# SamuelSchlesinger/anonymous-credit-tokens

Hardware: AMD Instinct MI355X
Metric: spend-proof verifies/sec (whole node), batch=2^20 (higher is better)
Workload: dtype u32 limbs / u64 accumulators (integer)

## Files before the change

anonymous-credit-tokens_amd/csrc/msm.h:

```cpp
#pragma once
#include "ge25519.h"

namespace act {

#ifndef ACT_FB_WBITS
#define ACT_FB_WBITS 16
#endif
constexpr int FB_WBITS = ACT_FB_WBITS;
constexpr int FB_WINDOWS = (253 + FB_WBITS - 1) / FB_WBITS;
constexpr int FB_ENTRIES = 1 << FB_WBITS;
constexpr int NIELS_WORDS = 32;
constexpr size_t FB_TABLE_WORDS = (size_t)FB_WINDOWS * FB_ENTRIES * NIELS_WORDS;

ACT_HD ge_niels niels_load(const uint32_t* p) {
  ge_niels n;
#if defined(__HIP_DEVICE_COMPILE__)
  const uint4* q = reinterpret_cast<const uint4*>(p);
  uint4 a[7];
  for (int i = 0; i < 7; i++) a[i] = q[i];
  uint32_t w[28];
  for (int i = 0; i < 7; i++) { w[4 * i] = a[i].x; w[4 * i + 1] = a[i].y; w[4 * i + 2] = a[i].z; w[4 * i + 3] = a[i].w; }
  for (int i = 0; i < FE_LIMBS; i++) { n.ypx.v[i] = w[i]; n.ymx.v[i] = w[FE_LIMBS + i]; n.xy2d.v[i] = w[2 * FE_LIMBS + i]; }
#else
  for (int i = 0; i < FE_LIMBS; i++) { n.ypx.v[i] = p[i]; n.ymx.v[i] = p[FE_LIMBS + i]; n.xy2d.v[i] = p[2 * FE_LIMBS + i]; }
#endif
  return n;
}
ACT_HD void niels_store(uint32_t* p, const ge_niels& n) {
  for (int i = 0; i < FE_LIMBS; i++) { p[i] = n.ypx.v[i]; p[FE_LIMBS + i] = n.ymx.v[i]; p[2 * FE_LIMBS + i] = n.xy2d.v[i]; }
  for (int i = 3 * FE_LIMBS; i < NIELS_WORDS; i++) p[i] = 0;
}
ACT_HD ge_niels niels_from_affine(const ge& p) {
  ge_niels n;
  n.ypx = fe_carry(fe_add(p.Y, p.X));
  n.ymx = fe_carry(fe_sub(p.Y, p.X));
  n.xy2d = fe_mul(p.T, fe_d2());
  return n;
}
constexpr int GE_WORDS = 4 * FE_LIMBS;
ACT_HD void ge_words(uint32_t w[GE_WORDS], const ge& g) {
  for (int i = 0; i < FE_LIMBS; i++) { w[i] = g.X.v[i]; w[FE_LIMBS + i] = g.Y.v[i]; w[2 * FE_LIMBS + i] = g.Z.v[i]; w[3 * FE_LIMBS + i] = g.T.v[i]; }
}
ACT_HD ge ge_of_words(const uint32_t w[GE_WORDS]) {
  ge g;
  for (int i = 0; i < FE_LIMBS; i++) { g.X.v[i] = w[i]; g.Y.v[i] = w[FE_LIMBS + i]; g.Z.v[i] = w[2 * FE_LIMBS + i]; g.T.v[i] = w[3 * FE_LIMBS + i]; }
  return g;
}
ACT_HD void ge_store(uint32_t* p, const ge& g) { ge_words(p, g); }
ACT_HD ge ge_load(const uint32_t* p) { return ge_of_words(p); }

struct FbTab { const uint32_t* p; uint32_t wbits; uint32_t id; };
ACT_HD uint32_t fb_windows(uint32_t wbits) { return (253u + wbits - 1u) / wbits; }
ACT_HD size_t fb_table_words(uint32_t wbits) { return (size_t)fb_windows(wbits) * ((size_t)1 << wbits) * NIELS_WORDS; }

ACT_HD ge_niels fb_table_entry(ge b, uint32_t wbits, uint32_t gid) {
  uint32_t pos = gid >> wbits, e = gid & ((1u << wbits) - 1u);
  for (uint32_t i = 0; i < wbits * pos; i++) b = ge_double(b);
  ge acc = ge_identity();
  ge_cached bc = ge_to_cached(b);
  for (int bit = (int)wbits - 1; bit >= 0; bit--) {
    acc = ge_double(acc);
    if ((e >> bit) & 1u) acc = ge_add_cached(acc, bc);
  }
  fe zi = fe_invert(acc.Z);
  ge af; af.X = fe_mul(acc.X, zi); af.Y = fe_mul(acc.Y, zi); af.Z = fe_one(); af.T = fe_mul(af.X, af.Y);
  return niels_from_affine(af);
}

ACT_HD uint32_t fb_next_digit(uint32_t w[8], uint32_t wbits) {
  uint32_t digit = w[0] & ((1u << wbits) - 1u);
  for (int i = 0; i < 7; i++) w[i] = (w[i] >> wbits) | (w[i + 1] << (32u - wbits));
  w[7] >>= wbits;
  return digit;
}
ACT_HD ge fixed_base_acc(ge acc, const FbTab& t, const sc& s) {
  fe_count_fixed_base(t.id);
  uint32_t w[8];
  for (int i = 0; i < 8; i++) w[i] = s.v[i];
  const uint32_t nw = fb_windows(t.wbits);
  const size_t entries = (size_t)1 << t.wbits;
  ge_niels cur = niels_load(t.p + (size_t)fb_next_digit(w, t.wbits) * NIELS_WORDS);
  for (uint32_t pos = 1; pos < nw; pos++) {
    ge_niels nxt = niels_load(t.p + ((size_t)pos * entries + fb_next_digit(w, t.wbits)) * NIELS_WORDS);
    acc = ge_madd(acc, cur);
    cur = nxt;
  }
  return ge_madd(acc, cur);
}

struct digit4 { bool nonzero, two, neg; };
ACT_HD digit4 next_digit4(uint32_t w[8], uint32_t& carry) {
  uint32_t v = (w[0] & 3u) + carry;
  for (int i = 0; i < 7; i++) w[i] = (w[i] >> 2) | (w[i + 1] << 30);
  w[7] >>= 2;
  digit4 d;
  carry = v >= 3u ? 1u : 0u;
  d.nonzero = (v != 0u) && (v != 4u);
  d.two = (v == 2u);
  d.neg = (v == 3u);
  return d;
}
ACT_HD ge chain_step_add(const ge& acc, const ge_cached& c1, const ge_cached& c2, const digit4& d) {
  ge_cached q;
  uint32_t m2 = fe_mask(d.two);
  q.YpX = fe_select_m(c1.YpX, c2.YpX, m2);
  q.YmX = fe_select_m(c1.YmX, c2.YmX, m2);
  q.Z = fe_select_m(c1.Z, c2.Z, m2);
  q.T2d = fe_select_m(c1.T2d, c2.T2d, m2);
  q = ge_cached_cneg(q, d.neg);
  return ge_add_cached(acc, q);
}
template <int NACC>
ACT_HD void chain(ge* acc, const ge& N, const sc* s) {
  uint32_t w[NACC][8], carry[NACC];
  for (int a = 0; a < NACC; a++) { carry[a] = 0; for (int i = 0; i < 8; i++) w[a][i] = s[a].v[i]; }
  ge P = N;
  for (int step = 0; step < 127; step++) {
    ge_cached c1 = ge_to_cached(P);
    ge Q = ge_double(P);
    ge_cached c2 = ge_to_cached(Q);
    if (step < 126) P = ge_double(Q);
#pragma unroll
    for (int a = 0; a < NACC; a++) {
      digit4 d = next_digit4(w[a], carry[a]);
      if (d.nonzero) acc[a] = chain_step_add(acc[a], c1, c2, d);
    }
  }
}

struct naf_state { uint32_t w[9]; };
ACT_HD naf_state naf_init(const sc& s) { naf_state n; for (int i = 0; i < 8; i++) n.w[i] = s.v[i]; n.w[8] = 0; return n; }
ACT_HD int naf_next(naf_state& n) {
  int d = 0;
  if (n.w[0] & 1u) {
    d = 2 - (int)(n.w[0] & 3u);
    if (d < 0) {
      uint64_t c = 1;
      for (int i = 0; i < 9; i++) { c += n.w[i]; n.w[i] = (uint32_t)c; c >>= 32; }
    } else {
      n.w[0] &= ~1u;
    }
  }
  for (int i = 0; i < 8; i++) n.w[i] = (n.w[i] >> 1) | (n.w[i + 1] << 31);
  n.w[8] >>= 1;
  return d;
}
ACT_HD int naf3_next(naf_state& n) {
  int d = 0;
  if (n.w[0] & 1u) {
    const uint32_t m = n.w[0] & 7u;
    d = m < 4u ? (int)m : (int)m - 8;
    n.w[0] &= ~7u;
    if (d < 0) {
      uint64_t c = 8;
      for (int i = 0; i < 9; i++) { c += n.w[i]; n.w[i] = (uint32_t)c; c >>= 32; }
    }
  }
  for (int i = 0; i < 8; i++) n.w[i] = (n.w[i] >> 1) | (n.w[i + 1] << 31);
  n.w[8] >>= 1;
  return d;
}
ACT_HD void chain2u(ge& acc_l, ge& acc_u, const ge& N, const sc& s_l, const sc& s_u) {
  uint32_t w[8], carry = 0;
  for (int i = 0; i < 8; i++) w[i] = s_l.v[i];
  naf_state nu = naf_init(s_u);
  ge P = N;
  for (int step = 0; step < 127; step++) {
    ge_cached c1 = ge_to_cached(P);
    ge Q = ge_double(P);
    ge_cached c2 = ge_to_cached(Q);
    if (step < 126) P = ge_double(Q);
    digit4 d = next_digit4(w, carry);
    if (d.nonzero) acc_l = chain_step_add(acc_l, c1, c2, d);
    int u0 = naf_next(nu);
    if (u0 != 0) acc_u = ge_add_cached(acc_u, ge_cached_cneg(c1, u0 < 0));
    int u1 = naf_next(nu);
    if (u1 != 0) acc_u = ge_add_cached(acc_u, ge_cached_cneg(c2, u1 < 0));
  }
}

constexpr int BUCKETS = 9;
constexpr int BUCKET_WORDS = BUCKETS * GE_WORDS;

constexpr int GE_PIECES = GE_WORDS / 4;
ACT_HD ge bucket_load(const uint32_t* p) {
#if defined(__HIP_DEVICE_COMPILE__)
  const uint4* q = reinterpret_cast<const uint4*>(p);
  uint4 a[GE_PIECES];
  for (int i = 0; i < GE_PIECES; i++) a[i] = q[i];
  uint32_t w[GE_WORDS];
  for (int i = 0; i < GE_PIECES; i++) { w[4 * i] = a[i].x; w[4 * i + 1] = a[i].y; w[4 * i + 2] = a[i].z; w[4 * i + 3] = a[i].w; }
  return ge_of_words(w);
#else
  return ge_load(p);
#endif
}
ACT_HD void bucket_store(uint32_t* p, const ge& g) {
#if defined(__HIP_DEVICE_COMPILE__)
  uint32_t w[GE_WORDS];
  ge_words(w, g);
  uint4* q = reinterpret_cast<uint4*>(p);
  for (int i = 0; i < GE_PIECES; i++) q[i] = make_uint4(w[4 * i], w[4 * i + 1], w[4 * i + 2], w[4 * i + 3]);
#else
  ge_store(p, g);
#endif
}
constexpr int GE_LDS_WORDS_PER_WAVE = GE_PIECES * 64 * 4;

#if defined(__HIP_DEVICE_COMPILE__)
__device__ __forceinline__ void ge_to_lds(uint32_t* lds_wave, const ge& g) {
  const uint32_t lane = threadIdx.x & 63u;
  uint32_t w[GE_WORDS];
  ge_words(w, g);
  for (int k = 0; k < GE_PIECES; k++)
    *reinterpret_cast<uint4*>(lds_wave + (k * 64 + lane) * 4) = make_uint4(w[4 * k], w[4 * k + 1], w[4 * k + 2], w[4 * k + 3]);
}
__device__ __forceinline__ ge ge_from_lds(const uint32_t* lds_wave) {
  const uint32_t lane = threadIdx.x & 63u;
  uint32_t w[GE_WORDS];
  for (int k = 0; k < GE_PIECES; k++) {
    const uint4 q = *reinterpret_cast<const uint4*>(lds_wave + (k * 64 + lane) * 4);
    w[4 * k] = q.x; w[4 * k + 1] = q.y; w[4 * k + 2] = q.z; w[4 * k + 3] = q.w;
  }
  return ge_of_words(w);
}
#endif

constexpr int NAF_WORDS = 64;
ACT_HD void naf3_recode(uint32_t out[NAF_WORDS], const sc& s) {
  naf_state n = naf_init(s);
  for (int step = 0; step < NAF_WORDS; step++) {
    uint32_t wd = 0;
    for (int k = 0; k < 4; k++) wd |= ((uint32_t)naf3_next(n) & 0xffu) << (8 * k);
    out[step] = wd;
  }
}
ACT_HD void radix16_bias(uint32_t t[8], const sc& s) {
  uint64_t c = 0;
  for (int i = 0; i < 8; i++) { c += (uint64_t)s.v[i] + 0x88888888u; t[i] = (uint32_t)c; c >>= 32; }
}
ACT_HD int naf_byte(uint32_t wd, int k) { return (int)(int8_t)(wd >> (8 * k)); }

template <bool UNIFORM>
ACT_HD void chain_bu_pre(ge& acc_l, ge& acc_u, const ge& N, const uint32_t* dg, const uint32_t* nafw, uint32_t* bk, uint32_t* lds_wave = nullptr, bool n_small = false) {
  const ge id = ge_identity();
  uint32_t touched = 0;
#if defined(__HIP_DEVICE_COMPILE__)
  ge_to_lds(lds_wave, id);
  ge_to_lds(lds_wave + GE_LDS_WORDS_PER_WAVE, id);
  auto add_u = [&](const ge_ded& q, int d) {
    uint32_t* home = lds_wave + ((d == 3 || d == -3) ? GE_LDS_WORDS_PER_WAVE : 0);
    ge_to_lds(home, ge_add_ded(ge_from_lds(home), ge_ded_cneg(q, d < 0)));
  };
#else
  ge U[2] = {id, id};
  auto add_u = [&](const ge_ded& q, int d) {
    ge& t = U[(d == 3 || d == -3) ? 1 : 0];
    t = ge_add_ded(t, ge_ded_cneg(q, d < 0));
  };
#endif
  ge P = N;
  uint32_t dw = 0;
#if defined(ACT_BUCKET_PREFETCH)
  ge Bpre = id;
  uint32_t nib_next = dg[0] & 15u;
#endif
  for (int step = 0; step < 64; step++) {
#if defined(ACT_BUCKET_PREFETCH)
    if ((step & 7) == 0) dw = dg[step >> 3] >> 4;
    const uint32_t nib = nib_next;
#else
    if ((step & 7) == 0) dw = dg[step >> 3];
    const uint32_t nib = dw & 15u; dw >>= 4;
#endif
    const bool neg = nib < 8u;
    const uint32_t mag = neg ? 8u - nib : nib - 8u;
    uint32_t nw = nafw[step];
#if defined(__HIP_DEVICE_COMPILE__)
    if (UNIFORM) nw = (uint32_t)__builtin_amdgcn_readfirstlane((int)nw);
#endif
    const int u = naf_byte(nw, 0), u1 = naf_byte(nw, 1), u2 = naf_byte(nw, 2), u3 = naf_byte(nw, 3);
    ge_ded c = ge_to_ded(P);
    uint32_t* slot = bk + mag * GE_WORDS;
    if (mag != 0u) {
#if defined(ACT_BUCKET_PREFETCH)
      ge B = Bpre;
#else
      ge B = id;
      if ((touched >> mag) & 1u) B = bucket_load(slot);
#endif
      touched |= 1u << mag;
      B = ge_add_ded(B, ge_ded_cneg(c, neg));
      bucket_store(slot, B);
    }
    if (u != 0) add_u(c, u);
    if (step == 63) {
      if (u1 != 0) { P = ge_double_opt(P, true); add_u(ge_to_ded(P), u1); }
      break;
    }
    P = ge_double_opt(P, u1 != 0);
    if (u1 != 0) add_u(ge_to_ded(P), u1);
    P = ge_double_opt(P, u2 != 0);
    if (u2 != 0) add_u(ge_to_ded(P), u2);
    P = ge_double_opt(P, u3 != 0);
    if (u3 != 0) add_u(ge_to_ded(P), u3);
#if defined(ACT_BUCKET_PREFETCH)
    {
      if (((step + 1) & 7) == 0) nib_next = dg[(step + 1) >> 3] & 15u; else { nib_next = dw & 15u; dw >>= 4; }
      const uint32_t mag_next = nib_next < 8u ? 8u - nib_next : nib_next - 8u;
      Bpre = id;
      if (mag_next != 0u && ((touched >> mag_next) & 1u)) Bpre = bucket_load(bk + mag_next * GE_WORDS);
    }
#endif
    P = ge_double_opt(P, true);
  }
  {
#if defined(__HIP_DEVICE_COMPILE__)
    ge U1 = ge_from_lds(lds_wave), U3 = ge_from_lds(lds_wave + GE_LDS_WORDS_PER_WAVE);
#else
    ge U1 = U[0], U3 = U[1];
#endif
    const uint32_t ms = fe_mask(n_small);
    U1 = ge_select_m(U1, id, ms); U3 = ge_select_m(U3, id, ms);
    acc_u = ge_add_cached(acc_u, ge_to_cached(U1));
    acc_u = ge_add_cached(acc_u, ge_to_cached(U3));
    acc_u = ge_add_cached(acc_u, ge_to_cached(ge_double_opt(U3, true)));
  }
  auto bucket = [&](int vv) { ge B = id; if ((touched >> vv) & 1u) B = bucket_load(bk + vv * GE_WORDS); return B; };
  ge S = bucket(8);
  ge R = S;
  for (int vv = 7; vv >= 1; vv--) {
    S = ge_add_cached(S, ge_to_cached(bucket(vv)));
    R = ge_add_cached(R, ge_to_cached(S));
  }
  acc_l = ge_select_m(R, id, fe_mask(n_small));
}

ACT_HD void chain_bu(ge& acc_l, ge& acc_u, const ge& N, const sc& s_l, const sc& s_u, uint32_t* bk, uint32_t* lds_wave = nullptr) {
  const ge id = ge_identity();
  for (int b = 0; b < BUCKETS; b++) bucket_store(bk + b * GE_WORDS, id);
  uint32_t w[8], carry = 0;
  for (int i = 0; i < 8; i++) w[i] = s_l.v[i];
  naf_state nu = naf_init(s_u);
#if defined(__HIP_DEVICE_COMPILE__)
  ge_to_lds(lds_wave, id);
  ge_to_lds(lds_wave + GE_LDS_WORDS_PER_WAVE, id);
  auto add_u = [&](const ge_cached& q, int d) {
    uint32_t* home = lds_wave + ((d == 3 || d == -3) ? GE_LDS_WORDS_PER_WAVE : 0);
    ge_to_lds(home, ge_add_cached(ge_from_lds(home), ge_cached_cneg(q, d < 0)));
  };
#else
  ge U[2] = {id, id};
  auto add_u = [&](const ge_cached& q, int d) {
    ge& t = U[(d == 3 || d == -3) ? 1 : 0];
    t = ge_add_cached(t, ge_cached_cneg(q, d < 0));
  };
#endif
  ge P = N;
  for (int step = 0; step < 64; step++) {
    uint32_t v = (w[0] & 15u) + carry;
    for (int i = 0; i < 7; i++) w[i] = (w[i] >> 4) | (w[i + 1] << 28);
    w[7] >>= 4;
    carry = v > 8u ? 1u : 0u;
    bool neg = v > 8u;
    uint32_t mag = neg ? 16u - v : v;
    ge_cached c = ge_to_cached(P);
    uint32_t* slot = bk + mag * GE_WORDS;
    ge B = bucket_load(slot);
    B = ge_add_cached(B, ge_cached_cneg(c, neg));
    bucket_store(slot, B);
    int u = naf3_next(nu);
    if (u != 0) add_u(c, u);
    int u1 = naf3_next(nu), u2 = naf3_next(nu), u3 = naf3_next(nu);
    if (step == 63) {
      if (u1 != 0) { P = ge_double_opt(P, true); add_u(ge_to_cached(P), u1); }
      break;
    }
    P = ge_double_opt(P, u1 != 0);
    if (u1 != 0) add_u(ge_to_cached(P), u1);
    P = ge_double_opt(P, u2 != 0);
    if (u2 != 0) add_u(ge_to_cached(P), u2);
    P = ge_double_opt(P, u3 != 0);
    if (u3 != 0) add_u(ge_to_cached(P), u3);
    P = ge_double_opt(P, true);
  }
  {
#if defined(__HIP_DEVICE_COMPILE__)
    const ge U1 = ge_from_lds(lds_wave), U3 = ge_from_lds(lds_wave + GE_LDS_WORDS_PER_WAVE);
#else
    const ge U1 = U[0], U3 = U[1];
#endif
    acc_u = ge_add_cached(acc_u, ge_to_cached(U1));
    acc_u = ge_add_cached(acc_u, ge_to_cached(U3));
    acc_u = ge_add_cached(acc_u, ge_to_cached(ge_double_opt(U3, true)));
  }
  ge S = bucket_load(bk + 8 * GE_WORDS);
  ge R = S;
  for (int vv = 7; vv >= 1; vv--) {
    S = ge_add_cached(S, ge_to_cached(bucket_load(bk + vv * GE_WORDS)));
    R = ge_add_cached(R, ge_to_cached(S));
  }
  acc_l = R;
}

template <int NACC>
ACT_HD void chain_b(ge* acc, const ge& N, const sc* s, uint32_t* bk) {
  const ge id = ge_identity();
  for (int b = 0; b < NACC * BUCKETS; b++) bucket_store(bk + b * GE_WORDS, id);
  uint32_t w[NACC][8], carry[NACC];
  for (int a = 0; a < NACC; a++) { carry[a] = 0; for (int i = 0; i < 8; i++) w[a][i] = s[a].v[i]; }
  ge P = N;
  for (int step = 0; step < 64; step++) {
    ge_cached c = ge_to_cached(P);
#pragma unroll
    for (int a = 0; a < NACC; a++) {
      uint32_t v = (w[a][0] & 15u) + carry[a];
      for (int i = 0; i < 7; i++) w[a][i] = (w[a][i] >> 4) | (w[a][i + 1] << 28);
      w[a][7] >>= 4;
      carry[a] = v > 8u ? 1u : 0u;
      bool neg = v > 8u;
      uint32_t mag = neg ? 16u - v : v;
      uint32_t* slot = bk + ((size_t)a * BUCKETS + mag) * GE_WORDS;
      bucket_store(slot, ge_add_cached(bucket_load(slot), ge_cached_cneg(c, neg)));
    }
    if (step == 63) break;
    P = ge_double_opt(P, false); P = ge_double_opt(P, false); P = ge_double_opt(P, false);
    P = ge_double_opt(P, true);
  }
  for (int a = 0; a < NACC; a++) {
    const uint32_t* ba = bk + (size_t)a * BUCKET_WORDS;
    ge S = bucket_load(ba + 8 * GE_WORDS);
    ge R = S;
    for (int vv = 7; vv >= 1; vv--) {
      S = ge_add_cached(S, ge_to_cached(bucket_load(ba + vv * GE_WORDS)));
      R = ge_add_cached(R, ge_to_cached(S));
    }
    acc[a] = ge_add_cached(acc[a], ge_to_cached(R));
  }
}

constexpr int CT_WINDOWS = 64, CT_ENTRIES = 8;
constexpr size_t CT_TABLE_WORDS = (size_t)CT_WINDOWS * CT_ENTRIES * NIELS_WORDS;
ACT_HD ge fixed_base_acc_ct(ge acc, const uint32_t* table, const sc& s) {
  uint32_t t[8];
  radix16_bias(t, s);
#pragma unroll 1
  for (int wd = 0; wd < 8; wd++) {
    uint32_t word = t[0];
    for (int i = 0; i < 7; i++) t[i] = t[i + 1];
#pragma unroll 1
    for (int k = 0; k < 8; k++) {
      const uint32_t nib = word & 15u; word >>= 4;
      const bool neg = nib < 8u;
      const uint32_t mag = neg ? 8u - nib : nib - 8u;
      const uint32_t* row = table + (size_t)(wd * 8 + k) * CT_ENTRIES * NIELS_WORDS;
      ge_niels q = ge_niels_identity();
      for (uint32_t e = 1; e <= (uint32_t)CT_ENTRIES; e++) {
        const ge_niels c = niels_load(row + (size_t)(e - 1) * NIELS_WORDS);
        const uint32_t m = fe_mask(e == mag);
        q.ypx = fe_select_m(q.ypx, c.ypx, m); q.ymx = fe_select_m(q.ymx, c.ymx, m); q.xy2d = fe_select_m(q.xy2d, c.xy2d, m);
      }
      acc = ge_madd(acc, ge_niels_cneg(q, neg));
    }
  }
  return acc;
}
#ifndef ACT_MF_KSTEPS
#define ACT_MF_KSTEPS 2
#endif
constexpr int MF_KSTEPS = ACT_MF_KSTEPS, MF_ENTRIES = 32 * MF_KSTEPS;
constexpr int MF_WBITS = MF_KSTEPS == 1 ? 6 : MF_KSTEPS == 2 ? 7 : 8, MF_WINDOWS = (253 + MF_WBITS - 1) / MF_WBITS;
constexpr int MF_WINDOW_BYTES = MF_KSTEPS * 4 * 2 * 32 * 16;
static_assert(MF_KSTEPS == 1 || MF_KSTEPS == 2 || MF_KSTEPS == 4, "32, 64 or 128 entries per window");
#if defined(__HIP_DEVICE_COMPILE__)
typedef int mf_v4i __attribute__((ext_vector_type(4)));
typedef int mf_v16i __attribute__((ext_vector_type(16)));
__device__ __forceinline__ mf_v4i mf_onehot16(int idx, int h) {
  const int rel = idx - 16 * h;
  const int val = (int)(1u << (8 * (rel & 3))), w = rel >> 2;
  mf_v4i b;
  b[0] = (w == 0) ? val : 0; b[1] = (w == 1) ? val : 0; b[2] = (w == 2) ? val : 0; b[3] = (w == 3) ? val : 0;
  return b;
}
__device__ __forceinline__ uint32_t mf_pack4(const mf_v16i& v, int q) {
  return __builtin_amdgcn_perm((uint32_t)v[4 * q + 1], (uint32_t)v[4 * q], 0x0c0c0400u) |
         (__builtin_amdgcn_perm((uint32_t)v[4 * q + 3], (uint32_t)v[4 * q + 2], 0x0c0c0400u) << 16);
}
__device__ __forceinline__ void mf_select(uint32_t w[27], const uint8_t* tabA, int idx) {
  const int lane = (int)(threadIdx.x & 63u), h = lane >> 5, r = lane & 31;
  const auto sw = __builtin_amdgcn_permlane32_swap((unsigned)idx, (unsigned)idx, false, false);
  mf_v4i b_lo[MF_KSTEPS], b_hi[MF_KSTEPS];
#pragma unroll
  for (int ks = 0; ks < MF_KSTEPS; ks++) { b_lo[ks] = mf_onehot16((int)sw[0] - 32 * ks, h); b_hi[ks] = mf_onehot16((int)sw[1] - 32 * ks, h); }
  const mf_v16i zero = {0, 0, 0, 0, 0, 0, 0, 0, 0, 0, 0, 0, 0, 0, 0, 0};
#pragma unroll
  for (int t = 0; t < 4; t++) {
    mf_v16i x = zero, y = zero;
#pragma unroll
    for (int ks = 0; ks < MF_KSTEPS; ks++) {
      const mf_v4i a = *reinterpret_cast<const mf_v4i*>(tabA + (((ks * 4 + t) * 2 + h) * 32 + r) * 16);
      x = __builtin_amdgcn_mfma_i32_32x32x32_i8(a, b_lo[ks], x, 0, 0, 0);
      y = __builtin_amdgcn_mfma_i32_32x32x32_i8(a, b_hi[ks], y, 0, 0, 0);
    }
    const int nq = t < 3 ? 4 : 2;
#pragma unroll
    for (int q = 0; q < nq; q++) {
      const bool need_hi = t < 3 || q == 0;
      uint32_t xw = mf_pack4(x, q), yw = mf_pack4(y, q);
      const auto s = __builtin_amdgcn_permlane32_swap(xw, yw, false, false);
      w[8 * t + 2 * q] = s[0];
      if (need_hi) w[8 * t + 2 * q + 1] = s[1];
    }
  }
}
__device__ __forceinline__ constexpr uint32_t mf_bias_word(int i) {
  uint32_t v = 0;
  for (int w = 0; w < MF_WINDOWS; w++) { const int bit = MF_WBITS * w + MF_WBITS - 1; if (bit / 32 == i) v |= 1u << (bit % 32); }
  return v;
}
__device__ __forceinline__ ge fixed_base_acc_mf(ge acc, const uint8_t* tab_mf, const sc& s) {
  uint32_t t[9];
  uint64_t c = 0;
  constexpr uint32_t bias[9] = {mf_bias_word(0), mf_bias_word(1), mf_bias_word(2), mf_bias_word(3), mf_bias_word(4), mf_bias_word(5), mf_bias_word(6), mf_bias_word(7), mf_bias_word(8)};
  for (int i = 0; i < 8; i++) { c += (uint64_t)s.v[i] + bias[i]; t[i] = (uint32_t)c; c >>= 32; }
  t[8] = (uint32_t)c + bias[8];
#pragma unroll 1
  for (int wd = 0; wd < MF_WINDOWS; wd++) {
    const int d = (int)(t[0] & ((1u << MF_WBITS) - 1u)) - (1 << (MF_WBITS - 1));
    for (int i = 0; i < 8; i++) t[i] = (t[i] >> MF_WBITS) | (t[i + 1] << (32 - MF_WBITS));
    t[8] >>= MF_WBITS;
    const bool neg = d < 0;
    const int mag = neg ? -d : d;
    uint32_t w[27];
    mf_select(w, tab_mf + (size_t)wd * MF_WINDOW_BYTES, mag - 1);
    const uint32_t one = mag == 0 ? 1u : 0u;
    ge_niels q;
    for (int i = 0; i < FE_LIMBS; i++) { q.ypx.v[i] = w[i]; q.ymx.v[i] = w[FE_LIMBS + i]; q.xy2d.v[i] = w[2 * FE_LIMBS + i]; }
    q.ypx.v[0] |= one; q.ymx.v[0] |= one;
    acc = ge_madd(acc, ge_niels_cneg(q, neg));
  }
  return acc;
}
#elif defined(__HIPCC__)
__device__ ge fixed_base_acc_mf(ge acc, const uint8_t* tab_mf, const sc& s);
#endif

template <int NACC>
ACT_HD void chain_ct(ge* acc, const ge& N, const sc* s, int steps = 127) {
  uint32_t w[NACC][8], carry[NACC];
  for (int a = 0; a < NACC; a++) { carry[a] = 0; for (int i = 0; i < 8; i++) w[a][i] = s[a].v[i]; }
  ge_cached idc; idc.YpX = fe_one(); idc.YmX = fe_one(); idc.Z = fe_one(); idc.T2d = fe_zero();
  ge P = N;
#pragma unroll 1
  for (int step = 0; step < steps; step++) {
    ge_cached c1 = ge_to_cached(P);
    ge Q = ge_double(P);
    ge_cached c2 = ge_to_cached(Q);
    if (step < steps - 1) P = ge_double(Q);
#pragma unroll
    for (int a = 0; a < NACC; a++) {
      digit4 d = next_digit4(w[a], carry[a]);
      const uint32_t m2 = fe_mask(d.two), mz = fe_mask(!d.nonzero);
      ge_cached q;
      q.YpX = fe_select_m(c1.YpX, c2.YpX, m2); q.YmX = fe_select_m(c1.YmX, c2.YmX, m2);
      q.Z = fe_select_m(c1.Z, c2.Z, m2); q.T2d = fe_select_m(c1.T2d, c2.T2d, m2);
      q = ge_cached_cneg(q, d.neg);
      q.YpX = fe_select_m(q.YpX, idc.YpX, mz); q.YmX = fe_select_m(q.YmX, idc.YmX, mz);
      q.Z = fe_select_m(q.Z, idc.Z, mz); q.T2d = fe_select_m(q.T2d, idc.T2d, mz);
      acc[a] = ge_add_cached(acc[a], q);
    }
  }
}
ACT_HD ge chain_ct_quarter(const ge& N, const sc& s, int i) {
  ge P = N;
#pragma unroll 1
  for (int d = 0; d < 64 * i; d++) P = ge_double(P);
  sc piece = sc_zero();
  piece.v[0] = s.v[2 * i]; piece.v[1] = s.v[2 * i + 1];
  ge acc[1] = {ge_identity()};
  sc sp[1] = {piece};
  chain_ct<1>(acc, P, sp, 33);
  return acc[0];
}
#if defined(ACT_CT_SECRET_TABLES)
template <int NACC> ACT_HD void chain_s(ge* acc, const ge& N, const sc* s, uint32_t*) { chain_ct<NACC>(acc, N, s); }
#else
template <int NACC> ACT_HD void chain_s(ge* acc, const ge& N, const sc* s, uint32_t* bk) { chain_b<NACC>(acc, N, s, bk); }
#endif

template <int E, typename Slot, typename Emit>
ACT_HD void dc_encode_batch(int count, Slot slot, Emit emit) {
  fe prefix[E];
  fe acc = fe_one();
#pragma unroll
  for (int i = 0; i < E; i++) {
    if (i < count) {
      uint32_t* w = slot(i);
      dc_efgh s = dc_prepare(bucket_load(w));
      ge t; t.X = s.e; t.Y = s.f; t.Z = s.g; t.T = s.h; bucket_store(w, t);
      fe eg, fh; bool z;
      fe prod = dc_product(eg, fh, z, s);
      prefix[i] = acc;
      acc = fe_mul(acc, prod);
    }
  }
  fe inv = fe_invert(acc);
#pragma unroll
  for (int i = E - 1; i >= 0; i--) {
    if (i < count) {
      ge t = bucket_load(slot(i));
      dc_efgh s; s.e = t.X; s.f = t.Y; s.g = t.Z; s.h = t.T;
      fe eg, fh; bool z;
      fe prod = dc_product(eg, fh, z, s);
      fe mine = fe_select(fe_mul(inv, prefix[i]), fe_zero(), z);
      inv = fe_mul(inv, prod);
      uint32_t enc[8];
      dc_finish(enc, s, eg, fh, mine);
      emit(i, enc);
    }
  }
}

}
```

anonymous-credit-tokens_amd/csrc/spend_lanes.h:

```cpp
#pragma once
#include "kernels.h"

namespace act {

#if defined(__HIP_DEVICE_COMPILE__) && defined(ACT_PIECES_NOINLINE)
#define ACT_PIECE __device__ __attribute__((noinline))
#else
#define ACT_PIECE ACT_HD
#endif

constexpr int ENC_BATCH = 32;

ACT_PIECE ge spend_prep_role_a(const SpendArgs& a, uint32_t p, uint32_t& flags) {
  const ProofLayout pl{a.P.L};
  const SpendTranscript st{a.P.L};
  const uint8_t* rec = a.proofs + (size_t)p * pl.bytes();
  uint8_t* el = a.tr + (size_t)p * a.tr_stride + 184;
  uint32_t wk[8], wa[8];
  load8(wk, rec + 32 * pl.k()); load8(wa, rec + 32 * pl.a_prime());
  ge A;
  if (!ristretto_decode(A, wa)) flags |= FLAG_UNDECODABLE;
  if (ristretto_is_identity(A)) flags |= FLAG_IDENTITY;
  sc k = sc_from_words(wk);
  tr_put_aligned(el + 40 * st.el_k(), k.v);
  tr_put_aligned(el + 40 * st.el_a_prime(), wa);
  sc gamma = load_sc(rec + 32 * pl.gamma()), e_bar = load_sc(rec + 32 * pl.e_bar());
  ge acc[1] = {ge_identity()};
  sc sa[1] = {sc_sub(e_bar, sc_mul(a.K.x, gamma))};
  chain_ct<1>(acc, A, sa);
  return acc[0];
}
ACT_PIECE void spend_prep_role_b(const SpendArgs& a, uint32_t p, uint32_t& flags, ge& a1b, ge& a2b) {
  const ProofLayout pl{a.P.L};
  const SpendTranscript st{a.P.L};
  const uint8_t* rec = a.proofs + (size_t)p * pl.bytes();
  uint8_t* el = a.tr + (size_t)p * a.tr_stride + 184;
  uint32_t wb[8];
  load8(wb, rec + 32 * pl.b_bar());
  ge B;
  if (!ristretto_decode(B, wb)) flags |= FLAG_UNDECODABLE;
  tr_put_aligned(el + 40 * st.el_b_bar(), wb);
  ge acc[2] = {ge_identity(), ge_identity()};
  sc sb[2] = {load_sc(rec + 32 * pl.r2_bar()), load_sc(rec + 32 * pl.r3_bar())};
  chain_b<2>(acc, B, sb, a.pbk + ((size_t)p * PREP_BUCKET_SETS + 1) * BUCKET_WORDS);
  a1b = acc[0]; a2b = acc[1];
}
ACT_PIECE ge spend_prep_role_c_a2(const SpendArgs& a, uint32_t p) {
  const ProofLayout pl{a.P.L};
  const uint8_t* rec = a.proofs + (size_t)p * pl.bytes();
  tr_put_prefix(a.tr + (size_t)p * a.tr_stride, a.P, LABEL_SPEND);
  if (a.bind) tr_put_bind(a.tr + (size_t)p * a.tr_stride, a.P.L, a.bind + (size_t)p * 32);
  sc k = load_sc(rec + 32 * pl.k()), gamma = load_sc(rec + 32 * pl.gamma());
  sc c_bar = load_sc(rec + 32 * pl.c_bar()), r_bar = load_sc(rec + 32 * pl.r_bar());
  sc ngamma = sc_neg(gamma);
  ge f = fixed_base_acc(ge_identity(), a.P.tab[BASE_H1], c_bar);
  f = fixed_base_acc(f, a.P.tab[BASE_H3], r_bar);
  f = fixed_base_acc(f, a.P.tab[BASE_G], ngamma);
  return fixed_base_acc(f, a.P.tab[BASE_H2], sc_mul(ngamma, k));
}
ACT_PIECE void spend_prep_role_c_bits(const SpendArgs& a, uint32_t p) {
  const ProofLayout pl{a.P.L};
  const uint8_t* rec = a.proofs + (size_t)p * pl.bytes();
  sc gamma = load_sc(rec + 32 * pl.gamma());
  sc w00 = load_sc(rec + 32 * pl.w00()), w01 = load_sc(rec + 32 * pl.w01());
  ge d0 = fixed_base_acc(ge_identity(), a.P.tab[BASE_H2], sc_half(w00));
  ge d1 = fixed_base_acc(ge_identity(), a.P.tab[BASE_H2], sc_half(w01));
  ge_store(a.d01 + (size_t)p * 2 * GE_WORDS, d0);
  ge_store(a.d01 + (size_t)p * 2 * GE_WORDS + GE_WORDS, d1);
  naf3_recode(a.naf + (size_t)p * NAF_WORDS, sc_half(gamma));
}
ACT_PIECE ge spend_prep_role_c(const SpendArgs& a, uint32_t p) {
  ge f = spend_prep_role_c_a2(a, p);
  spend_prep_role_c_bits(a, p);
  return f;
}
ACT_PIECE void spend_prep_put(const SpendArgs& a, uint32_t p, int element, const ge& pt) {
  uint32_t enc[8];
  ristretto_encode(enc, pt);
  tr_put_aligned(a.tr + (size_t)p * a.tr_stride + 184 + 40 * element, enc);
}
ACT_HD void spend_prep_lane(const SpendArgs& a, uint32_t p) {
  const SpendTranscript st{a.P.L};
  uint32_t flags = 0;
  ge a1a = spend_prep_role_a(a, p, flags);
  ge a1b, a2b;
  spend_prep_role_b(a, p, flags, a1b, a2b);
  ge a2f = spend_prep_role_c(a, p);
  spend_prep_put(a, p, st.el_a1(), ge_add(a1a, a1b));
  spend_prep_put(a, p, st.el_a2(), ge_add(a2f, a2b));
  a.flags[p] = flags;
}

ACT_HD void spend_prep_a_lane(const SpendArgs& a, uint32_t p) {
  uint32_t flags = 0;
  ge_store(a.part + ((size_t)p * PART_POINTS + 0) * GE_WORDS, spend_prep_role_a(a, p, flags));
  if (flags) ACT_FLAG_OR(a.flags + p, flags);
}
ACT_HD void spend_prep_b_lane(const SpendArgs& a, uint32_t p) {
  uint32_t flags = 0;
  ge a1b, a2b;
  spend_prep_role_b(a, p, flags, a1b, a2b);
  ge_store(a.part + ((size_t)p * PART_POINTS + 1) * GE_WORDS, a1b);
  ge_store(a.part + ((size_t)p * PART_POINTS + 2) * GE_WORDS, a2b);
  if (flags) ACT_FLAG_OR(a.flags + p, flags);
}
ACT_HD void spend_prep_c_lane(const SpendArgs& a, uint32_t p) {
  ge_store(a.part + ((size_t)p * PART_POINTS + 3) * GE_WORDS, spend_prep_role_c(a, p));
}
ACT_HD void spend_prep_c1_lane(const SpendArgs& a, uint32_t p) { spend_prep_role_c_bits(a, p); }
ACT_HD void spend_prep_c2_lane(const SpendArgs& a, uint32_t p) {
  ge_store(a.part + ((size_t)p * PART_POINTS + 3) * GE_WORDS, spend_prep_role_c_a2(a, p));
}
ACT_HD void spend_prep_join_lane(const SpendArgs& a, uint32_t p) {
  const SpendTranscript st{a.P.L};
  const uint32_t* q = a.part + (size_t)p * PART_POINTS * GE_WORDS;
  spend_prep_put(a, p, st.el_a1(), ge_add(ge_load(q), ge_load(q + GE_WORDS)));
  spend_prep_put(a, p, st.el_a2(), ge_add(ge_load(q + 3 * GE_WORDS), ge_load(q + 2 * GE_WORDS)));
}
ACT_HD void spend_coords_lane(const SpendArgs& a, uint32_t gid) {
  const int L = a.P.L;
  uint32_t p = gid / (uint32_t)L, j = gid % (uint32_t)L;
  if (p >= a.n) return;
  const ProofLayout pl{L};
  uint32_t wc[8];
  load8(wc, a.proofs + (size_t)p * pl.bytes() + 32 * pl.com(j));
  ge C;
  if (!ristretto_decode(C, wc)) ACT_FLAG_OR(a.flags + p, FLAG_UNDECODABLE);
  niels_store(a.coords + ((size_t)p * L + j) * NIELS_WORDS, niels_from_affine(C));
}

template <bool UNIFORM>
ACT_HD void spend_bits_lane(const SpendArgs& a, uint32_t gid, uint32_t* lds_wave) {
  const int L = a.P.L;
  uint32_t p = gid / (uint32_t)L, j = gid % (uint32_t)L;
  if (p >= a.n) return;
  const ProofLayout pl{L};
  const SpendTranscript st{L};
  const uint8_t* rec = a.proofs + (size_t)p * pl.bytes();
  uint8_t* el = a.tr + (size_t)p * a.tr_stride + 184;

  uint32_t wc[8];
  load8(wc, rec + 32 * pl.com(j));
  ge C;
  bool ok = ristretto_decode(C, wc);
  if (!ok) ACT_FLAG_OR(a.flags + p, FLAG_UNDECODABLE);
  tr_put_aligned(el + 40 * st.el_com(j), wc);
  niels_store(a.coords + ((size_t)p * L + j) * NIELS_WORDS, niels_from_affine(C));

  sc gamma = sc_half(load_sc(rec + 32 * pl.gamma()));
  sc g0 = sc_half(load_sc(rec + 32 * pl.gamma0(j)));
  sc g1 = sc_sub(gamma, g0);
  sc z0 = sc_half(load_sc(rec + 32 * pl.z(j, 0))), z1 = sc_half(load_sc(rec + 32 * pl.z(j, 1)));

  ge acc_u = fixed_base_acc(ge_identity(), a.P.tab[BASE_H3], z1);
  acc_u = fixed_base_acc(acc_u, a.P.tab[BASE_H1], g1);
  if (j == 0) acc_u = ge_add(acc_u, ge_load(a.d01 + (size_t)p * 2 * GE_WORDS + GE_WORDS));
  ge acc_l = ge_identity();
#if defined(ACT_ABLATE_BUCKET_FOOTPRINT)
  uint32_t* bk = a.buckets + (size_t)(gid % ACT_ABLATE_BUCKET_FOOTPRINT) * BUCKET_WORDS;
#else
  uint32_t* bk = a.buckets + (size_t)gid * BUCKET_WORDS;
#endif
  uint32_t* dg = a.dig + (size_t)gid * 8;
  { uint32_t t[8]; radix16_bias(t, g0); for (int i = 0; i < 8; i++) dg[i] = t[i]; }
  const bool n_small = !ok || (wc[0] | wc[1] | wc[2] | wc[3] | wc[4] | wc[5] | wc[6] | wc[7]) == 0u;
  chain_bu_pre<UNIFORM>(acc_l, acc_u, ge_neg(C), dg, a.naf + (size_t)p * NAF_WORDS, bk, lds_wave, n_small);
  ge f0 = fixed_base_acc(ge_identity(), a.P.tab[BASE_H3], z0);
  if (j == 0) f0 = ge_add(f0, ge_load(a.d01 + (size_t)p * 2 * GE_WORDS));
  ge_cached dl = ge_to_cached(acc_l);
  bucket_store(bk, ge_add_cached(f0, dl));
  bucket_store(bk + GE_WORDS, ge_add_cached(acc_u, ge_cached_cneg(dl, true)));
}

constexpr int ENC_BATCH_SMALL = 8;
template <int E>
ACT_HD void spend_enc_lane_e(const SpendArgs& a, uint64_t q0) {
  const uint32_t L = (uint32_t)a.P.L;
  const uint64_t total = (uint64_t)a.n * L * 2u;
  if (q0 >= total) return;
  const int count = (int)(total - q0 < (uint64_t)E ? total - q0 : (uint64_t)E);
  const SpendTranscript st{a.P.L};
  dc_encode_batch<E>(
      count,
      [&](int i) { uint64_t q = q0 + (uint64_t)i; return a.buckets + (size_t)(q >> 1) * BUCKET_WORDS + (q & 1u) * GE_WORDS; },
      [&](int i, const uint32_t* enc) {
        uint64_t q = q0 + (uint64_t)i, lane = q >> 1;
        uint32_t p = (uint32_t)(lane / L), j = (uint32_t)(lane % L);
        tr_put_aligned(a.tr + (size_t)p * a.tr_stride + 184 + 40 * st.el_cprime(j, (int)(q & 1u)), enc);
      });
}
ACT_HD void spend_enc_lane(const SpendArgs& a, uint64_t q0) { spend_enc_lane_e<ENC_BATCH>(a, q0); }

ACT_HD ge spend_tail_horner(const SpendArgs& a, uint32_t p, int j_lo, int j_hi, int shift) {
  const int L = a.P.L;
  ge kp = ge_identity();
  for (int j = j_hi - 1; j >= j_lo; j--) {
    kp = ge_double(kp);
    kp = ge_madd(kp, niels_load(a.coords + ((size_t)p * L + j) * NIELS_WORDS));
  }
  for (int i = 0; i < shift; i++) kp = ge_double(kp);
  return kp;
}
ACT_HD ge spend_tail_fixed(const SpendArgs& a, uint32_t p) {
  const ProofLayout pl{a.P.L};
  const uint8_t* rec = a.proofs + (size_t)p * pl.bytes();
  sc gamma = load_sc(rec + 32 * pl.gamma());
  sc s = load_sc(rec + 32 * pl.s()), c_bar = load_sc(rec + 32 * pl.c_bar());
  sc k_bar = load_sc(rec + 32 * pl.k_bar()), s_bar = load_sc(rec + 32 * pl.s_bar());
  ge f = fixed_base_acc(ge_identity(), a.P.tab[BASE_H1], sc_sub(sc_mul(sc_neg(gamma), s), c_bar));
  f = fixed_base_acc(f, a.P.tab[BASE_H2], k_bar);
  return fixed_base_acc(f, a.P.tab[BASE_H3], s_bar);
}
ACT_HD void spend_tail_c(const SpendArgs& a, uint32_t p, const ge& kp, const ge& f) {
  const ProofLayout pl{a.P.L};
  const SpendTranscript st{a.P.L};
  ge acc[1] = {f};
  sc sk_[1] = {sc_neg(load_sc(a.proofs + (size_t)p * pl.bytes() + 32 * pl.gamma()))};
  chain_b<1>(acc, kp, sk_, a.pbk + (size_t)p * PREP_BUCKET_SETS * BUCKET_WORDS);
  uint32_t enc[8];
  ristretto_encode(enc, acc[0]); tr_put_aligned(a.tr + (size_t)p * a.tr_stride + 184 + 40 * st.el_c(), enc);
}
ACT_HD void spend_tail_xa(const SpendArgs& a, uint32_t p, const ge& kp) {
  ge_store(a.xa + (size_t)p * GE_WORDS, ge_add(kp, ge_basepoint()));
  if (a.kprime_enc) { uint32_t enc[8]; ristretto_encode(enc, kp); store8(a.kprime_enc + (size_t)p * 32, enc); }
}
ACT_HD void spend_tail_lane(const SpendArgs& a, uint32_t p) {
  ge kp = spend_tail_horner(a, p, 0, a.P.L, 0);
  spend_tail_c(a, p, kp, spend_tail_fixed(a, p));
  spend_tail_xa(a, p, kp);
}
ACT_HD void spend_tail_k_lane(const SpendArgs& a, uint32_t p) { spend_tail_xa(a, p, spend_tail_horner(a, p, 0, a.P.L, 0)); }
ACT_HD void spend_tail_c_lane(const SpendArgs& a, uint32_t p) {
  const ge kp = ge_add(ge_load(a.xa + (size_t)p * GE_WORDS), ge_neg(ge_basepoint()));
  spend_tail_c(a, p, kp, spend_tail_fixed(a, p));
}

ACT_HD void spend_finish_lane(const SpendArgs& a, uint32_t p) {
  const ProofLayout pl{a.P.L};
  sc gamma = load_sc(a.proofs + (size_t)p * pl.bytes() + 32 * pl.gamma());
  uint32_t w[16];
  for (int i = 0; i < 16; i++) w[i] = a.xof[(size_t)p * 16 + i];
  sc chal = sc_from_wide_words(w);
  uint32_t f = a.flags[p];
  uint8_t stt = 0;
  if (f & FLAG_UNDECODABLE) stt = 255;
  else if (f & FLAG_IDENTITY) stt = 6;
  else if (!sc_equal(chal, gamma)) stt = 7;
  a.status[p] = stt;
  if (a.kprime_enc && stt != 0) zero8(a.kprime_enc + (size_t)p * 32);
}

}
```

Baseline: 518,700.

## Slice bucket combine, fold sums into fixed-base accumulators, pick lightest NAF representative

The radix-16 bucket reduction now uses a bit-sliced form: buckets are grouped by bit and combined with three doublings. This replaces the serial running-sum chain with fewer point additions. The fixed-base accumulations now start from the chain outputs, so the final additions and the cached conversions are folded in. The NAF recode for gamma/2 now tries s, s+l, l-s and 2l-s, keeping the one with the fewest nonzero digits (negated when needed). This cuts additions in the upper chain but adds four full weight scans in prep, and the sign handling has to be correct.

```diff
diff --git a/anonymous-credit-tokens_amd/csrc/msm.h b/anonymous-credit-tokens_amd/csrc/msm.h
--- a/anonymous-credit-tokens_amd/csrc/msm.h
+++ b/anonymous-credit-tokens_amd/csrc/msm.h
@@ -235,13 +235,50 @@
     out[step] = wd;
   }
 }
+ACT_HD int naf3_weigh(const uint32_t v[8]) {
+  naf_state n; for (int i = 0; i < 8; i++) n.w[i] = v[i]; n.w[8] = 0;
+  int nz = 0;
+  for (int pos = 0; pos < 253; pos++) nz += naf3_next(n) != 0 ? 1 : 0;
+  uint32_t rest = 0;
+  for (int i = 0; i < 9; i++) rest |= n.w[i];
+  return rest != 0u ? -1 : nz;
+}
+ACT_HD int naf3_recode_lightest(uint32_t out[NAF_WORDS], const sc& s) {
+  uint32_t l[8], l2[8], cand[8], best[8];
+  for (int i = 0; i < 8; i++) { l[i] = sc_l_word(i); best[i] = s.v[i]; }
+  bn_add<8>(l2, l, l);
+  int best_i = 0, best_w = naf3_weigh(s.v);
+  if (best_w < 0) best_w = 4 * NAF_WORDS;
+  for (int c = 1; c < 4; c++) {
+    if (c == 1) bn_add<8>(cand, s.v, l); else if (c == 2) bn_sub<8>(cand, l, s.v); else bn_sub<8>(cand, l2, s.v);
+    const int w = naf3_weigh(cand);
+    if (w >= 0 && w < best_w) { best_w = w; best_i = c; for (int i = 0; i < 8; i++) best[i] = cand[i]; }
+  }
+  naf_state n; for (int i = 0; i < 8; i++) n.w[i] = best[i]; n.w[8] = 0;
+  const bool neg = best_i >= 2;
+  for (int step = 0; step < NAF_WORDS; step++) {
+    uint32_t wd = 0;
+    for (int k = 0; k < 4; k++) { const int d = naf3_next(n); wd |= ((uint32_t)(neg ? -d : d) & 0xffu) << (8 * k); }
+    out[step] = wd;
+  }
+  return best_i;
+}
 ACT_HD void radix16_bias(uint32_t t[8], const sc& s) {
   uint64_t c = 0;
   for (int i = 0; i < 8; i++) { c += (uint64_t)s.v[i] + 0x88888888u; t[i] = (uint32_t)c; c >>= 32; }
 }
 ACT_HD int naf_byte(uint32_t wd, int k) { return (int)(int8_t)(wd >> (8 * k)); }
 
-template <bool UNIFORM>
+#ifndef ACT_BITS_SLICED_COMBINE
+#define ACT_BITS_SLICED_COMBINE 1
+#endif
+#ifndef ACT_BITS_FOLD_SUMS
+#define ACT_BITS_FOLD_SUMS 1
+#endif
+#ifndef ACT_BITS_LIGHT_NAF
+#define ACT_BITS_LIGHT_NAF 1
+#endif
+template <bool UNIFORM, bool FOLD = false>
 ACT_HD void chain_bu_pre(ge& acc_l, ge& acc_u, const ge& N, const uint32_t* dg, const uint32_t* nafw, uint32_t* bk, uint32_t* lds_wave = nullptr, bool n_small = false) {
   const ge id = ge_identity();
   uint32_t touched = 0;
@@ -314,26 +351,53 @@
 #endif
     P = ge_double_opt(P, true);
   }
-  {
+  const uint32_t ms = fe_mask(n_small);
+  if (!FOLD) {
 #if defined(__HIP_DEVICE_COMPILE__)
     ge U1 = ge_from_lds(lds_wave), U3 = ge_from_lds(lds_wave + GE_LDS_WORDS_PER_WAVE);
 #else
     ge U1 = U[0], U3 = U[1];
 #endif
-    const uint32_t ms = fe_mask(n_small);
     U1 = ge_select_m(U1, id, ms); U3 = ge_select_m(U3, id, ms);
     acc_u = ge_add_cached(acc_u, ge_to_cached(U1));
     acc_u = ge_add_cached(acc_u, ge_to_cached(U3));
     acc_u = ge_add_cached(acc_u, ge_to_cached(ge_double_opt(U3, true)));
   }
   auto bucket = [&](int vv) { ge B = id; if ((touched >> vv) & 1u) B = bucket_load(bk + vv * GE_WORDS); return B; };
+#if ACT_BITS_SLICED_COMBINE
+  ge R;
+  {
+    const ge_cached c7 = ge_to_cached(bucket(7));
+    const ge_cached c67 = ge_to_cached(ge_add_cached(bucket(6), c7));
+    const ge_cached c5 = ge_to_cached(bucket(5));
+    R = ge_double_opt(bucket(8), true);
+    R = ge_add_cached<false>(R, ge_to_cached(ge_add_cached(ge_add_cached(bucket(4), c5), c67)));
+    const ge_cached c3 = ge_to_cached(bucket(3));
+    R = ge_double_opt(R, true);
+    R = ge_add_cached<false>(R, ge_to_cached(ge_add_cached(ge_add_cached(bucket(2), c3), c67)));
+    R = ge_double_opt(R, true);
+    R = ge_add_cached(R, ge_to_cached(ge_add_cached(ge_add_cached(ge_add_cached(bucket(1), c3), c5), c7)));
+  }
+#else
   ge S = bucket(8);
   ge R = S;
   for (int vv = 7; vv >= 1; vv--) {
     S = ge_add_cached(S, ge_to_cached(bucket(vv)));
     R = ge_add_cached(R, ge_to_cached(S));
   }
-  acc_l = ge_select_m(R, id, fe_mask(n_small));
+#endif
+  acc_l = ge_select_m(R, id, ms);
+  if (FOLD) {
+#if defined(__HIP_DEVICE_COMPILE__)
+    ge U1 = ge_from_lds(lds_wave), U3 = ge_from_lds(lds_wave + GE_LDS_WORDS_PER_WAVE);
+#else
+    ge U1 = U[0], U3 = U[1];
+#endif
+    U1 = ge_select_m(U1, id, ms); U3 = ge_select_m(U3, id, ms);
+    ge G = ge_add_cached(U1, ge_to_cached(U3));
+    G = ge_add_cached(G, ge_to_cached(ge_double_opt(U3, true)));
+    acc_u = ge_add_cached(G, ge_cached_cneg(ge_to_cached(acc_l), true));
+  }
 }
 
 ACT_HD void chain_bu(ge& acc_l, ge& acc_u, const ge& N, const sc& s_l, const sc& s_u, uint32_t* bk, uint32_t* lds_wave = nullptr) {
diff --git a/anonymous-credit-tokens_amd/csrc/spend_lanes.h b/anonymous-credit-tokens_amd/csrc/spend_lanes.h
--- a/anonymous-credit-tokens_amd/csrc/spend_lanes.h
+++ b/anonymous-credit-tokens_amd/csrc/spend_lanes.h
@@ -67,7 +67,11 @@
   ge d1 = fixed_base_acc(ge_identity(), a.P.tab[BASE_H2], sc_half(w01));
   ge_store(a.d01 + (size_t)p * 2 * GE_WORDS, d0);
   ge_store(a.d01 + (size_t)p * 2 * GE_WORDS + GE_WORDS, d1);
+#if ACT_BITS_LIGHT_NAF
+  naf3_recode_lightest(a.naf + (size_t)p * NAF_WORDS, sc_half(gamma));
+#else
   naf3_recode(a.naf + (size_t)p * NAF_WORDS, sc_half(gamma));
+#endif
 }
 ACT_PIECE ge spend_prep_role_c(const SpendArgs& a, uint32_t p) {
   ge f = spend_prep_role_c_a2(a, p);
@@ -152,9 +156,13 @@
   sc g1 = sc_sub(gamma, g0);
   sc z0 = sc_half(load_sc(rec + 32 * pl.z(j, 0))), z1 = sc_half(load_sc(rec + 32 * pl.z(j, 1)));
 
+#if ACT_BITS_FOLD_SUMS == 0
   ge acc_u = fixed_base_acc(ge_identity(), a.P.tab[BASE_H3], z1);
   acc_u = fixed_base_acc(acc_u, a.P.tab[BASE_H1], g1);
   if (j == 0) acc_u = ge_add(acc_u, ge_load(a.d01 + (size_t)p * 2 * GE_WORDS + GE_WORDS));
+#else
+  ge acc_u = ge_identity();
+#endif
   ge acc_l = ge_identity();
 #if defined(ACT_ABLATE_BUCKET_FOOTPRINT)
   uint32_t* bk = a.buckets + (size_t)(gid % ACT_ABLATE_BUCKET_FOOTPRINT) * BUCKET_WORDS;
@@ -164,12 +172,23 @@
   uint32_t* dg = a.dig + (size_t)gid * 8;
   { uint32_t t[8]; radix16_bias(t, g0); for (int i = 0; i < 8; i++) dg[i] = t[i]; }
   const bool n_small = !ok || (wc[0] | wc[1] | wc[2] | wc[3] | wc[4] | wc[5] | wc[6] | wc[7]) == 0u;
+#if ACT_BITS_FOLD_SUMS == 0
   chain_bu_pre<UNIFORM>(acc_l, acc_u, ge_neg(C), dg, a.naf + (size_t)p * NAF_WORDS, bk, lds_wave, n_small);
   ge f0 = fixed_base_acc(ge_identity(), a.P.tab[BASE_H3], z0);
   if (j == 0) f0 = ge_add(f0, ge_load(a.d01 + (size_t)p * 2 * GE_WORDS));
   ge_cached dl = ge_to_cached(acc_l);
   bucket_store(bk, ge_add_cached(f0, dl));
   bucket_store(bk + GE_WORDS, ge_add_cached(acc_u, ge_cached_cneg(dl, true)));
+#else
+  chain_bu_pre<UNIFORM, true>(acc_l, acc_u, ge_neg(C), dg, a.naf + (size_t)p * NAF_WORDS, bk, lds_wave, n_small);
+  ge f0 = fixed_base_acc(acc_l, a.P.tab[BASE_H3], z0);
+  if (j == 0) f0 = ge_add(f0, ge_load(a.d01 + (size_t)p * 2 * GE_WORDS));
+  bucket_store(bk, f0);
+  acc_u = fixed_base_acc(acc_u, a.P.tab[BASE_H3], z1);
+  acc_u = fixed_base_acc(acc_u, a.P.tab[BASE_H1], g1);
+  if (j == 0) acc_u = ge_add(acc_u, ge_load(a.d01 + (size_t)p * 2 * GE_WORDS + GE_WORDS));
+  bucket_store(bk + GE_WORDS, acc_u);
+#endif
 }
 
 constexpr int ENC_BATCH_SMALL = 8;
```

Measured after the change: 519,600 (median of 6 runs). Within noise of the previous version (+0.2%).
